# bhargav0410/gpu-accel-ofdm-ls-mrc

Hardware: AMD Instinct MI355X
Metric: OFDM symbols/s (LS+MRC) at 1024 subcarriers x 64 ant; achieved HBM GB/s vs peak (higher is better)
Workload: dtype f32; 1 GPU; OFDM uplink LS+MRC, time-domain IQ in HBM, 1250 frames x 101 symbols (1 pilot + 100 data) x 64 antennas x 1024 subcarriers per GPU; domain=time, R=64, C=1024, S=101, prefix=0, frames_per_gpu=1250, data_symbols_per_gpu=125000, global_data_symbols=125000, flow=one-launch, parallelism=frame-sharded x1, no collective

## Files before the change

### gpu-accel-ofdm-ls-mrc_amd/csrc/common.hpp

```cpp
#pragma once
#include <hip/hip_runtime.h>
#include <stdint.h>

#include "twiddles.inc"

namespace ofdm {

__constant__ __attribute__((aligned(16))) float g_twf[2 * OFDM_TW_N] = {OFDM_TW_TABLE};
#define g_tw (reinterpret_cast<const float2 *>(g_twf))
struct TwTable { float v[2 * OFDM_TW_N]; };
constexpr TwTable kTw = {{OFDM_TW_TABLE}};

template <int N, int K>
__device__ __forceinline__ constexpr float2 tw_const() {
    static_assert(OFDM_TW_N % N == 0, "N must divide 4096");
    constexpr int idx = ((K % N + N) % N) * (OFDM_TW_N / N);
    return float2{kTw.v[2 * idx], kTw.v[2 * idx + 1]};
}

__device__ __forceinline__ int lane_here() {
    int l;
    asm volatile("v_mbcnt_lo_u32_b32 %0, -1, 0\n\tv_mbcnt_hi_u32_b32 %0, -1, %0" : "=v"(l));
    return l;
}

__device__ __forceinline__ float2 cadd(float2 a, float2 b) { return {a.x + b.x, a.y + b.y}; }
__device__ __forceinline__ float2 csub(float2 a, float2 b) { return {a.x - b.x, a.y - b.y}; }
__device__ __forceinline__ float2 cmul(float2 a, float2 b) {
    return {a.x * b.x - a.y * b.y, a.x * b.y + a.y * b.x};
}
__device__ __forceinline__ float2 cconj(float2 a) { return {a.x, -a.y}; }
template <bool INV>
__device__ __forceinline__ float2 cmul_mi(float2 a) {
    return INV ? float2{-a.y, a.x} : float2{a.y, -a.x};
}
template <bool INV>
__device__ __forceinline__ float2 tw_apply(float2 a, float2 w) {
    return cmul(a, INV ? cconj(w) : w);
}

template <int N>
__device__ __forceinline__ constexpr int bitrev(int i) {
    int r = 0;
    for (int b = 1, rb = N >> 1; b < N; b <<= 1, rb >>= 1)
        if (i & b) r |= rb;
    return r;
}

template <int N, bool INV>
__device__ __forceinline__ void fft_reg(float2 (&a)[N]) {
#pragma unroll
    for (int i = 0; i < N; ++i) {
        const int j = bitrev<N>(i);
        if (i < j) { float2 t = a[i]; a[i] = a[j]; a[j] = t; }
    }
#pragma unroll
    for (int len = 2; len <= N; len <<= 1) {
        const int half = len >> 1;
#pragma unroll
        for (int i = 0; i < N; i += len) {
#pragma unroll
            for (int k = 0; k < half; ++k) {
                float2 u = a[i + k], v = a[i + k + half];
                if (k == 0) {
                } else if (4 * k == len) {
                    v = cmul_mi<INV>(v);
                } else {
                    const int idx = k * (OFDM_TW_N / len);
                    float2 w{kTw.v[2 * idx], kTw.v[2 * idx + 1]};
                    v = tw_apply<INV>(v, w);
                }
                a[i + k] = cadd(u, v);
                a[i + k + half] = csub(u, v);
            }
        }
    }
}

template <int LOG2C, bool INV>
__device__ float2 *stockham_lds(float2 *a, float2 *b) {
    constexpr int C = 1 << LOG2C;
    constexpr int TWS = OFDM_TW_N / C;
    int Ns = 1;
#pragma unroll 1
    for (; Ns * 4 <= C; Ns *= 4) {
        for (int j = threadIdx.x; j < C / 4; j += blockDim.x) {
            const int k = j & (Ns - 1);
            float2 v0 = a[j], v1 = a[j + C / 4], v2 = a[j + C / 2], v3 = a[j + 3 * C / 4];
            const int t = k * (C / (4 * Ns));
            if (t) {
                v1 = tw_apply<INV>(v1, g_tw[t * TWS]);
                v2 = tw_apply<INV>(v2, g_tw[2 * t * TWS]);
                v3 = tw_apply<INV>(v3, g_tw[3 * t * TWS]);
            }
            const float2 s02 = cadd(v0, v2), d02 = csub(v0, v2);
            const float2 s13 = cadd(v1, v3), d13 = cmul_mi<INV>(csub(v1, v3));
            const int d = (j - k) * 4 + k;
            b[d] = cadd(s02, s13);
            b[d + Ns] = cadd(d02, d13);
            b[d + 2 * Ns] = csub(s02, s13);
            b[d + 3 * Ns] = csub(d02, d13);
        }
        __syncthreads();
        float2 *t = a; a = b; b = t;
    }
    if (Ns < C) {
        for (int j = threadIdx.x; j < C / 2; j += blockDim.x) {
            const int k = j & (Ns - 1);
            float2 v0 = a[j], v1 = a[j + C / 2];
            const int t = k * (C / (2 * Ns));
            if (t) v1 = tw_apply<INV>(v1, g_tw[t * TWS]);
            const int d = (j - k) * 2 + k;
            b[d] = cadd(v0, v1);
            b[d + Ns] = csub(v0, v1);
        }
        __syncthreads();
        float2 *t = a; a = b; b = t;
    }
    return a;
}

__device__ __forceinline__ int out_pos(int j, int K) {
    const int h = (K - 1) / 2;
    return j >= h ? j - h : j + (K + 1) / 2;
}
__device__ __forceinline__ int out_pos_any(int j, int K) {
    const int h = (K - 1) / 2, n2 = (K + 1) / 2;
    return j < h ? j + n2 : (j < h + n2 ? j - h : j);
}
__device__ __forceinline__ int out_src(int k, int K) {
    const int h = (K - 1) / 2, n2 = (K + 1) / 2;
    return k < n2 ? k + h : (k < n2 + h ? k - n2 : k);
}

__device__ __forceinline__ float2 ls_conj(float2 y, float2 x) {
    const float den = x.x * x.x + x.y * x.y;
    const float rd = __builtin_amdgcn_rcpf(den);
    const float re = (y.x * x.x + y.y * x.y) * rd;
    const float im = (y.y * x.x - y.x * x.y) * rd;
    return {re, -1.0f * im};
}

__device__ __forceinline__ uint64_t splitmix64(uint64_t z) {
    z += 0x9E3779B97F4A7C15ull;
    z = (z ^ (z >> 30)) * 0xBF58476D1CE4E5B9ull;
    z = (z ^ (z >> 27)) * 0x94D049BB133111EBull;
    return z ^ (z >> 31);
}
__device__ __forceinline__ uint64_t hash4(uint64_t seed, uint64_t a, uint64_t b, uint64_t c) {
    return splitmix64(splitmix64(splitmix64(seed ^ a) ^ b) ^ c);
}
__device__ __forceinline__ float u01(uint32_t x) {
    return ((float)(x >> 8) + 1.0f) * (1.0f / 16777216.0f);
}
__device__ __forceinline__ float2 gauss2(uint64_t h) {
    const float u1 = u01((uint32_t)h), u2 = u01((uint32_t)(h >> 32));
    const float rad = sqrtf(-2.0f * logf(u1));
    float s, c;
    sincosf(6.283185307179586f * u2, &s, &c);
    return {rad * c, rad * s};
}

}
```

### gpu-accel-ofdm-ls-mrc_amd/csrc/frame_td.hip

```cpp
#include "launch.hpp"
#include "wave_fft1024.hpp"
#include "diag.hpp"

OFDM_DIAG_TU(td1024)


namespace ofdm {
namespace td1024 {

constexpr int LS_WAVES = 4;

template <int NW>
__global__ void __launch_bounds__(64 * NW) k_ls_td1024(const float2 *__restrict__ iq, int S, int R,
                                                       int prefix, const float2 *__restrict__ X,
                                                       float2 *__restrict__ Hc, float *__restrict__ P,
                                                       int partial) {
    extern __shared__ __attribute__((aligned(16))) float2 lds[];
    float2 *tw = lds;
    const int w = threadIdx.x >> 6;
    const int t = threadIdx.x & 63;
    float2 *T = lds + TWBUF + w * TBUF;
    fill_twiddles(tw);
    __syncthreads();

    const long long f = blockIdx.x;
    const int Cp = C + prefix;
    const float2 *pilot = iq + f * (long long)S * R * Cp + prefix;
    float4 *Hf = reinterpret_cast<float4 *>(Hc + f * (long long)R * C);
    const int b0 = lane_bin0(t);
    float2 xp[16];
#pragma unroll
    for (int k = 0; k < 16; ++k) {
        const int b = b0 + 16 * k;
        xp[k] = b > 0 ? X[b - 1] : float2{1.f, 0.f};
    }
    float p[16];
#pragma unroll
    for (int k = 0; k < 16; ++k) p[k] = 0.f;
    for (int r = w; r < R; r += NW) {
        float2 a[16], x[16];
        row_load(pilot + (long long)r * Cp, t, a);
        row_fft(a, t, T, tw, x);
#pragma unroll
        for (int k = 0; k < 16; ++k) {
            float2 h = ls_conj(x[k], xp[k]);
            if (b0 + 16 * k == 0) h = float2{0.f, 0.f};
            x[k] = h;
            p[k] = p[k] + (h.x * h.x) + (h.y * h.y);
        }
        hc_store(Hf + (long long)r * (C / 2), t, x);
    }
    __syncthreads();
    float *pp = reinterpret_cast<float *>(lds + TWBUF);
    static_assert(NW * C * sizeof(float) <= NW * TBUF * sizeof(float2), "partials fit the transpose images");
#pragma unroll
    for (int k = 0; k < 16; ++k) pp[w * C + b0 + 16 * k] = p[k];
    __syncthreads();
    float *Pf = P + f * C;
    const int nw = R < NW ? R : NW;
    for (int b = threadIdx.x; b < C; b += blockDim.x) {
        float sum = pp[b];
        for (int i = 1; i < nw; ++i) sum = sum + pp[i * C + b];
        Pf[b] = b == 0 ? (partial ? 0.f : 1.f) : sum;
    }
}



template <bool PREF>
__device__ __forceinline__ void hlds_row_pf(const float2 *next, const float4 *hrow, int t, float2 (&a)[16],
                                            float2 *T, const float2 *tw1, const float2 *tw2,
                                            const float4 *lo, const float4 *hi, float4 *mine,
                                            float2 (&acc)[16]) {
    using namespace hlds;
    float2 x[16];
    row_fft_a(a, t, T, tw1);
    const float4 hreg = hrow[threadIdx.x];
    __builtin_amdgcn_sched_barrier(0);
    if (PREF) row_load<true>(next, t, a);
    row_fft_b(t, T, tw2, x);
    lds_barrier();
    *mine = hreg;
    lds_barrier();
#pragma unroll
    for (int i = 0; i < 8; ++i) {
        const float4 v = i < 4 ? lo[i * 64] : hi[(i - 4) * TS];
        acc[2 * i].x = acc[2 * i].x + (x[2 * i].x * v.x - x[2 * i].y * v.y);
        acc[2 * i].y = acc[2 * i].y + (x[2 * i].x * v.y + x[2 * i].y * v.x);
        acc[2 * i + 1].x = acc[2 * i + 1].x + (x[2 * i + 1].x * v.z - x[2 * i + 1].y * v.w);
        acc[2 * i + 1].y = acc[2 * i + 1].y + (x[2 * i + 1].x * v.w + x[2 * i + 1].y * v.z);
    }
}

template <bool R0>
__device__ __forceinline__ void row0(const float2 *sym, int t, const float2 *T, float2 (&a)[16]) {
    if constexpr (R0) {
        asm volatile("s_waitcnt vmcnt(0)" ::: "memory");
#pragma unroll
        for (int m = 0; m < 16; ++m) a[m] = T[t + 64 * m];
    } else {
        row_load<true>(sym, t, a);
    }
}
__device__ __forceinline__ void row0_dma(const float2 *sym, int t, float2 *T) {
    const char *src = reinterpret_cast<const char *>(sym) + t * 16;
    const unsigned dst = lds_addr(T);
#pragma unroll
    for (int j = 0; j < 8; ++j) dma16(src + j * 1024, dst + j * 1024);
}

template <bool SHARED, bool R0 = false>
__device__ __forceinline__ void hlds_rows(const float2 *sym, int Cp, int R, const float4 *Hf, int t,
                                          float2 *T, const float2 *tw1, const float2 *tw2,
                                          float2 *T0, float4 *hfree, float2 (&acc)[16]) {
    using namespace hlds;
#pragma unroll
    for (int k = 0; k < 16; ++k) acc[k] = float2{0.f, 0.f};
    if constexpr (SHARED) {
        float2 a[16];
        row0<R0>(sym, t, T, a);
        const float4 *lo = hfree + t;
        const float4 *hi = hslot(T0, hfree, 256 + t);
        float4 *mine = hslot(T0, hfree, threadIdx.x);
        for (int r = 0; r + 1 < R; ++r)
            hlds_row_pf<true>(sym + (long long)(r + 1) * Cp, Hf + (long long)r * (C / 2), lane_here(), a, T, tw1,
                                   tw2, lo, hi, mine, acc);
        hlds_row_pf<false>(sym, Hf + (long long)(R - 1) * (C / 2), lane_here(), a, T, tw1, tw2, lo, hi, mine,
                           acc);
    } else {
        for (int r = 0; r < R; ++r) {
            float2 a[16], x[16], h[16];
            if (r == 0)
                row0<R0>(sym, t, T, a);
            else
                row_load<true>(sym + (long long)r * Cp, t, a);
            row_fft_a(a, t, T, tw1);
            row_fft_b(t, T, tw2, x);
            __builtin_amdgcn_sched_barrier(0);
            hc_load(Hf + (long long)r * (C / 2), t, h);
#pragma unroll
            for (int k = 0; k < 16; ++k) {
                acc[k].x = acc[k].x + (x[k].x * h[k].x - x[k].y * h[k].y);
                acc[k].y = acc[k].y + (x[k].x * h[k].y + x[k].y * h[k].x);
            }
        }
    }
}

__device__ __forceinline__ void hlds_epilogue(const float2 (&acc)[16], const float *P, long long f, long long q,
                                              int t, float2 *T, float2 *__restrict__ out, int mode) {
    const int b0 = lane_bin0(t);
    float2 *o = out + q * K;
    const float *Pf = P + f * C + b0;
    float pv[16];
    if ((mode & 1) == 0) {
#pragma unroll
        for (int k = 0; k < 16; ++k) pv[k] = Pf[16 * k];
    }
#pragma unroll
    for (int k = 0; k < 16; ++k) {
        const int b = b0 + 16 * k;
        float2 v = acc[k];
        int j = b - 1;
        if ((mode & 1) == 0) {
            const float rp = __builtin_amdgcn_rcpf(pv[k]);
            v = float2{acc[k].x * rp, acc[k].y * rp};
            j = out_pos(b > 0 ? b - 1 : 0, K);
        }
        if (b > 0) T[(j >> 6) * hlds::TP + (j & 63)] = v;
    }
    wave_lds_sync();
#pragma unroll
    for (int m = 0; m < 16; ++m) {
        const int j = t + 64 * m;
        if (j < K) {
            const float2 v = T[m * hlds::TP + t];
            __builtin_nontemporal_store(__builtin_bit_cast(unsigned long long, v),
                                        reinterpret_cast<unsigned long long *>(o + j));
        }
    }
}

template <bool R0>
__global__ void __attribute__((amdgpu_flat_work_group_size(512, 512), amdgpu_waves_per_eu(4, 4)))
k_mrc_td1024_hlds(const float2 *__restrict__ iq, int S, int R, int prefix, const float2 *__restrict__ Hc,
                  const float *__restrict__ P, float2 *__restrict__ out, long long nq, long long nblocks,
                  long long per_xcd, int mode) {
    using namespace hlds;
    constexpr int HW = WAVES;
    extern __shared__ __attribute__((aligned(16))) float2 lds[];
    float2 *tw1 = lds, *tw2 = lds + TW1S;
    const int w = __builtin_amdgcn_readfirstlane(threadIdx.x >> 6), t = threadIdx.x & 63;
    float2 *T = lds + TW1S + TW2S + w * TS;
    float2 *T0 = lds + TW1S + TW2S;
    float4 *hfree = reinterpret_cast<float4 *>(T0 + HW * TS);
    const long long pb = blockIdx.x;
    const long long lb = (pb & 7) * per_xcd + (pb >> 3);
    if (lb >= nblocks) return;

    const int nsym = S - 1;
    const long long qw = lb * HW + w;
    const bool store = qw < nq;
    const long long q = store ? qw : nq - 1;
    const long long f = q / nsym;
    const long long f0 = (lb * HW) / nsym;
    const long long fl = ((lb * HW + HW - 1 < nq ? lb * HW + HW - 1 : nq - 1)) / nsym;
    const int s = 1 + (int)(q % nsym);
    const int Cp = C + prefix;
    const float2 *sym = iq + (f * S + s) * (long long)R * Cp + prefix;
    if constexpr (R0) row0_dma(sym, t, T);
    fill(tw1, tw2);
    __syncthreads();

    float2 acc[16];
    if (f0 == fl)
        hlds_rows<true, R0>(sym, Cp, R, reinterpret_cast<const float4 *>(Hc + f0 * (long long)R * C), t, T,
                                 tw1, tw2, T0, hfree, acc);
    else
        hlds_rows<false, R0>(sym, Cp, R, reinterpret_cast<const float4 *>(Hc + f * (long long)R * C), t, T,
                                tw1, tw2, T0, hfree, acc);
    if (!store) return;
    hlds_epilogue(acc, P, f, q, t, T, out, mode);
}


__device__ __forceinline__ void hlds_ls_frame(const float2 *__restrict__ iq, int S, int R, int prefix,
                                              const float2 *__restrict__ X, float2 *Hc, float *P, long long f,
                                              int w, int t, float2 *T, float2 *T0, const float2 *tw1,
                                              const float2 *tw2, unsigned long long *mx = nullptr) {
    using namespace hlds;
    (void)mx;
    const int Cp = C + prefix;
    const float2 *pilot = iq + f * (long long)S * R * Cp + prefix;
    float4 *Hf = reinterpret_cast<float4 *>(Hc + f * (long long)R * C);
    const int b0 = lane_bin0(t);
    float2 xp[16];
#pragma unroll
    for (int k = 0; k < 16; ++k) {
        const int b = b0 + 16 * k;
        xp[k] = b > 0 ? X[b - 1] : float2{1.f, 0.f};
    }
    float p[16];
#pragma unroll
    for (int k = 0; k < 16; ++k) p[k] = 0.f;
    for (int r = w; r < R; r += WAVES) {
        float2 a[16], x[16];
        const int tl = lane_here();
        row_load<true>(pilot + (long long)r * Cp, tl, a);
        row_fft_a(a, tl, T, tw1);
        row_fft_b(tl, T, tw2, x);
#pragma unroll
        for (int k = 0; k < 16; ++k) {
            float2 h = ls_conj(x[k], xp[k]);
            if (b0 + 16 * k == 0) h = float2{0.f, 0.f};
            x[k] = h;
            p[k] = p[k] + (h.x * h.x) + (h.y * h.y);
        }
#pragma unroll
        for (int i = 0; i < 8; ++i) store16_wt(Hf, R * C * 8, (r * (C / 2) + i * 64 + tl) * 16, x[2 * i], x[2 * i + 1]);
        if (r == w) {
            OFDM_DIAG_MARKP(mx, 1)
        }
    }
    OFDM_DIAG_MARKP(mx, 2)
    __syncthreads();
    float *pp = reinterpret_cast<float *>(T0);
#pragma unroll
    for (int k = 0; k < 16; ++k) pp[w * C + b0 + 16 * k] = p[k];
    __syncthreads();
    float *Pf = P + f * C;
    const int nw = R < WAVES ? R : WAVES;
    for (int b = threadIdx.x; b < C; b += blockDim.x) {
        float sum = pp[b];
        for (int i = 1; i < nw; ++i) sum = sum + pp[i * C + b];
        const float v = b == 0 ? 1.f : sum;
        store4_wt(Pf + b, v);
    }
    OFDM_DIAG_MARKP(mx, 3)
    __syncthreads();
}

__device__ __forceinline__ void split_unit(const float2 *__restrict__ iq, int S, int R, int prefix, const float2 *Hc,
                                           const float *P, float2 *__restrict__ out, long long nq, long long q0, int w,
                                           int t, float2 *T, float2 *T0, const float2 *tw1, const float2 *tw2) {
    const int nsym = S - 1, Cp = C + prefix, hh = w >> 2, R0 = (R + 1) >> 1;
    const long long qw = q0 + (w & 3);
    const bool store = qw < nq;
    const long long q = store ? qw : nq - 1;
    const long long f = q / nsym;
    const int s = 1 + (int)(q % nsym);
    const float2 *sym = iq + (f * S + s) * (long long)R * Cp + prefix;
    const float4 *Hf = reinterpret_cast<const float4 *>(Hc + f * (long long)R * C);
    float2 acc[16];
#pragma unroll
    for (int k = 0; k < 16; ++k) acc[k] = float2{0.f, 0.f};
    const int r1 = hh ? R : R0;
    for (int r = hh ? R0 : 0; r < r1; ++r) {
        float2 a[16], x[16], h[16];
        row_load<true>(sym + (long long)r * Cp, t, a);
        hlds::row_fft_a(a, t, T, tw1);
        hlds::row_fft_b(t, T, tw2, x);
        __builtin_amdgcn_sched_barrier(0);
        hc_load(Hf + (long long)r * (C / 2), t, h);
#pragma unroll
        for (int k = 0; k < 16; ++k) {
            acc[k].x = acc[k].x + (x[k].x * h[k].x - x[k].y * h[k].y);
            acc[k].y = acc[k].y + (x[k].x * h[k].y + x[k].y * h[k].x);
        }
    }
    if (hh) {
#pragma unroll
        for (int k = 0; k < 16; ++k) T[k * hlds::TP + t] = acc[k];
    }
    __syncthreads();
    if (hh) return;
    const float2 *Tp = T0 + (w + 4) * hlds::TS;
#pragma unroll
    for (int k = 0; k < 16; ++k) {
        const float2 v = Tp[k * hlds::TP + t];
        acc[k] = float2{acc[k].x + v.x, acc[k].y + v.y};
    }
    if (store) hlds_epilogue(acc, P, f, q, t, T, out, 0);
}

__global__ void __attribute__((amdgpu_flat_work_group_size(512, 512), amdgpu_waves_per_eu(4, 4)))
k_demod_td1024(const float2 *__restrict__ iq, int S, int R, int prefix, const float2 *__restrict__ X, float2 *Hc,
               float *P, float2 *__restrict__ out, long long nq, long long nblocks, Tickets tk, long long k0, long long split, unsigned long long *flags, unsigned long long epoch,
               int nls, long long nframes, long long spin_ticks) {
    using namespace hlds;
    constexpr int HW = WAVES;
    extern __shared__ __attribute__((aligned(16))) float2 lds[];
    float2 *tw1 = lds, *tw2 = lds + TW1S;
    const int w = __builtin_amdgcn_readfirstlane(threadIdx.x >> 6), t = threadIdx.x & 63;
    float2 *T = lds + TW1S + TW2S + w * TS;
    float2 *T0 = lds + TW1S + TW2S;
    float4 *hfree = reinterpret_cast<float4 *>(T0 + HW * TS);
    OFDM_DIAG_BEGIN()

    const bool estimator = (int)blockIdx.x < nls;
    auto first_frame = [&](long long lb) { return (lb * HW) / (S - 1); };
    auto last_frame = [&](long long lb) { return ((lb * HW + HW - 1 < nq ? lb * HW + HW - 1 : nq - 1)) / (S - 1); };
    const int nsym = S - 1, Cp = C + prefix;
    auto sym_of = [&](long long lb) {
        const long long qw = lb * HW + w, q = qw < nq ? qw : nq - 1;
        return iq + ((q / nsym) * S + 1 + q % nsym) * (long long)R * Cp + prefix;
    };
    long long e0 = 1, e1 = 0, lb = 0;
    int um = 0;
    if (estimator) {
        e0 = e1 = blockIdx.x;
        if (e0 >= nframes) return;
        __builtin_amdgcn_s_setprio(3);
        fill(tw1, tw2);
        __syncthreads();
        OFDM_DIAG_MARKN(0)
    } else {
        FillRegs fr;
        fill_load(fr);
        lb = wg_take_unit(tk, nblocks, k0, (long long)blockIdx.x - nls, split,
                          reinterpret_cast<long long *>(hfree + 255));
        if (lb < 0) return;
        OFDM_DIAG_MARKN(0)
        um = (int)(lb & 3);
        lb >>= 2;
        fill_store(tw1, tw2, fr);
        const long long f0 = first_frame(lb), fl = last_frame(lb);
        if (!um) row0_dma(sym_of(lb), t, T);
        bool seen_before = false;
        if (threadIdx.x == 0)
            seen_before = __hip_atomic_load((gu64 *)(flags + f0), __ATOMIC_RELAXED, __HIP_MEMORY_SCOPE_AGENT) == epoch &&
                          __hip_atomic_load((gu64 *)(flags + fl), __ATOMIC_RELAXED, __HIP_MEMORY_SCOPE_AGENT) == epoch;
        OFDM_DIAG_MARKN(1)
        if (!consume_flags(flags, f0, fl, epoch, spin_ticks, reinterpret_cast<int *>(hfree), seen_before)) {
            asm volatile("s_waitcnt vmcnt(0)" ::: "memory");
            __syncthreads();
            e0 = f0;
            e1 = fl;
        }
    }
    for (long long ff = e0; ff <= e1; ++ff)
        hlds_ls_frame(iq, S, R, prefix, X, Hc, P, ff, w, t, T, T0, tw1, tw2, OFDM_DIAG_ARG);
    if (estimator) {
        OFDM_DIAG_MARK()
        publish_flag(flags + e0, epoch);
        OFDM_DIAG_END_SLOT(td1024, epoch);
        return;
    }
    if (e0 <= e1) {
        acquire_all();
        if (!um) row0_dma(sym_of(lb), t, T);
    }
    OFDM_DIAG_MARK()

    if (um) {
        split_unit(iq, S, R, prefix, Hc, P, out, nq, lb * HW + 4 * (um - 1), w, t, T, T0, tw1, tw2);
        OFDM_DIAG_END_SLOT(td1024, epoch);
        return;
    }
    const long long qw = lb * HW + w;
    const bool store = qw < nq;
    const long long q = store ? qw : nq - 1;
    const long long f = q / nsym;
    const long long f0 = first_frame(lb), fl = last_frame(lb);
    const float2 *sym = sym_of(lb);
    float2 acc[16];
    if (f0 == fl)
        hlds_rows<true, true>(sym, Cp, R, reinterpret_cast<const float4 *>(Hc + f0 * (long long)R * C), t, T,
                              tw1, tw2, T0, hfree, acc);
    else
        hlds_rows<false, true>(sym, Cp, R, reinterpret_cast<const float4 *>(Hc + f * (long long)R * C), t, T,
                               tw1, tw2, T0, hfree, acc);
    OFDM_DIAG_MARKN(2)
    if (store) hlds_epilogue(acc, P, f, q, lane_here(), T, out, 0);
    OFDM_DIAG_END_SLOT(td1024, epoch);
}

}

hipError_t launch_ls_td1024(const float2 *iq, long long nframes, int S, int R, int prefix,
                            const float2 *X, float2 *Hc, float *P, int partial, hipStream_t s) {
    using namespace td1024;
    if (nframes <= 0) return hipSuccess;
    if (nframes > 0x7fffffffll) return hipErrorInvalidValue;
    int nw = (nframes * LS_WAVES < 2048 && R > LS_WAVES) ? 16 : LS_WAVES;
    auto k16 = k_ls_td1024<16>;
    auto k4 = k_ls_td1024<LS_WAVES>;
    auto k8 = k16;
    if (nw == 16 || nw == 8) {
        auto kern = nw == 16 ? k16 : k8;
        const size_t lds = (TWBUF + nw * TBUF) * sizeof(float2);
        if (hipError_t e = opt_in_lds(reinterpret_cast<const void *>(kern), (int)lds); e != hipSuccess) return e;
        hipLaunchKernelGGL(kern, dim3((unsigned)nframes), dim3(64 * nw), lds, s, iq, S, R, prefix, X, Hc, P,
                           partial);
        return hipGetLastError();
    }
    const size_t lds = (TWBUF + LS_WAVES * TBUF) * sizeof(float2);
    hipLaunchKernelGGL(k4, dim3((unsigned)nframes), dim3(64 * LS_WAVES), lds, s, iq, S, R, prefix, X, Hc, P,
                       partial);
    return hipGetLastError();
}

hipError_t launch_mrc_td1024(const float2 *iq, long long nframes, int S, int R, int prefix,
                             const float2 *Hc, const float *P, float2 *out, int mode,
                             hipStream_t s) {
    using namespace td1024;
    const long long nq = nframes * (S - 1);
    if (nq <= 0) return hipSuccess;
    const long long nb = (nq + hlds::WAVES - 1) / hlds::WAVES;
    const long long pxcd = (nb + 7) / 8;
    if (pxcd * 8 > 0x7fffffffll) return hipErrorInvalidValue;
    auto kern = k_mrc_td1024_hlds<true>;
    hipLaunchKernelGGL(kern, dim3((unsigned)(pxcd * 8)), dim3(64 * hlds::WAVES), hlds::LDS_BYTES, s, iq, S, R,
                       prefix, Hc, P, out, nq, nb, pxcd, mode);
    return hipGetLastError();
}

hipError_t launch_demod_td1024(const float2 *iq, long long nframes, int S, int R, int prefix, const float2 *X,
                               float2 *Hc, float *P, float2 *out, Tickets tk,
                               unsigned long long *flags, unsigned long long epoch, long long spin_ticks,
                               hipStream_t s) {
    using namespace td1024;
    const long long nq = nframes * (S - 1);
    if (nq <= 0) return hipSuccess;
    const long long nb = (nq + hlds::WAVES - 1) / hlds::WAVES;
    const long long nls = (nframes + 7) / 8 * 8;
    const long long k1 = ticket_k0(2), k0 = 2 * k1, split = R >= 2 ? k1 : 0;
    const long long g = ticket_grid(nb, 8 * split);
    if (g + nls > 0x7fffffffll) return hipErrorInvalidValue;
    hipLaunchKernelGGL(k_demod_td1024, dim3((unsigned)(nls + g)), dim3(64 * hlds::WAVES), hlds::LDS_BYTES, s, iq,
                       S, R, prefix, X, Hc, P, out, nq, nb, tk, k0, split, flags, epoch, (int)nls, nframes,
                       spin_ticks < 0 ? SPIN_TICKS : spin_ticks);
    return hipGetLastError();
}

}
```

### gpu-accel-ofdm-ls-mrc_amd/csrc/wave_fft1024.hpp

```cpp
#pragma once
#include "common.hpp"
#include "launch.hpp"
#include "pk.hpp"

namespace ofdm {
namespace td1024 {

constexpr int C = 1024;
constexpr int K = C - 1;
constexpr int TP = 68;
constexpr int TBUF = 16 * TP;
constexpr int TW1P = 17;
constexpr int TW1BUF = 64 * TW1P;
constexpr int TW2P = 17;
constexpr int TW2BUF = 4 * TW2P;
constexpr int TWBUF = TW1BUF + TW2BUF;

__device__ __forceinline__ void wave_lds_sync() {
    __builtin_amdgcn_fence(__ATOMIC_RELEASE, "wavefront");
    __builtin_amdgcn_wave_barrier();
    __builtin_amdgcn_fence(__ATOMIC_ACQUIRE, "wavefront");
}

__device__ __forceinline__ void lds_barrier() {
    asm volatile("s_waitcnt lgkmcnt(0)\n\ts_barrier" ::: "memory");
}

typedef __attribute__((address_space(3))) void lvoid_t;
__device__ __forceinline__ unsigned lds_addr(const void *p) { return (unsigned)(size_t)(lvoid_t *)p; }

__device__ __forceinline__ void dma16(const void *g, unsigned lds) {
    unsigned keep;
    asm volatile("s_mov_b32 %0, m0\n\ts_mov_b32 m0, %2\n\ts_nop 0\n\tglobal_load_lds_dwordx4 %1, off\n\t"
                 "s_mov_b32 m0, %0"
                 : "=&s"(keep)
                 : "v"(g), "s"(lds)
                 : "memory");
}

__device__ __forceinline__ float quad_g(int a) { return (a == 0 || a == 3) ? 1.f : -1.f; }

__device__ __forceinline__ void fill_twiddles(float2 *tw) {
    for (int i = threadIdx.x; i < TW1BUF; i += blockDim.x) {
        const int t = i / TW1P, k2 = i % TW1P;
        tw[i] = k2 < 16 ? g_tw[((t * k2) & (C - 1)) * (OFDM_TW_N / C)] : float2{0.f, 0.f};
    }
    for (int i = threadIdx.x; i < TW2BUF; i += blockDim.x) {
        const int a = i / TW2P, k = i % TW2P;
        const float2 w = g_tw[((16 * a * k) & (C - 1)) * (OFDM_TW_N / C)];
        const float g = quad_g(a);
        tw[TW1BUF + i] = k < 16 ? float2{g * w.x, g * w.y} : float2{0.f, 0.f};
    }
}

template <int CTRL>
__device__ __forceinline__ float dpp(float v) {
    return __builtin_bit_cast(float, __builtin_amdgcn_mov_dpp(__builtin_bit_cast(int, v), CTRL,
                                                              0xF, 0xF, true));
}
constexpr int DPP_XOR1 = 0xB1;
constexpr int DPP_XOR2 = 0x4E;

template <bool NT = false>
__device__ __forceinline__ void row_load(const float2 *__restrict__ src, int t, float2 (&a)[16]) {
    if (NT) {
        const unsigned long long *p = reinterpret_cast<const unsigned long long *>(src) + t;
#pragma unroll
        for (int m = 0; m < 16; ++m)
            a[m] = __builtin_bit_cast(float2, __builtin_nontemporal_load(p + 64 * m));
    } else {
#pragma unroll
        for (int m = 0; m < 16; ++m) a[m] = src[t + 64 * m];
    }
}

#define OFDM_DPP_Q(CTRL) "quad_perm:" CTRL " row_mask:0xf bank_mask:0xf"
template <int CTRL>
__device__ __forceinline__ void quad_fmac_dpp(float (&v)[16], float S) {
#define OFDM_F(i) "v_fmac_f32_dpp %" #i ", %" #i ", %16 " OFDM_DPP_Q(QP) "\n\t"
    if constexpr (CTRL == 0x4E) {
#define QP "[2,3,0,1]"
        asm("s_nop 1\n\t" OFDM_F(0) OFDM_F(1) OFDM_F(2) OFDM_F(3) OFDM_F(4) OFDM_F(5) OFDM_F(6)
                OFDM_F(7) OFDM_F(8) OFDM_F(9) OFDM_F(10) OFDM_F(11) OFDM_F(12) OFDM_F(13) OFDM_F(14)
                    OFDM_F(15)
            : "+v"(v[0]), "+v"(v[1]), "+v"(v[2]), "+v"(v[3]), "+v"(v[4]), "+v"(v[5]), "+v"(v[6]),
              "+v"(v[7]), "+v"(v[8]), "+v"(v[9]), "+v"(v[10]), "+v"(v[11]), "+v"(v[12]),
              "+v"(v[13]), "+v"(v[14]), "+v"(v[15])
            : "v"(S));
#undef QP
    } else {
        static_assert(CTRL == 0xB1, "quad xor 1 or xor 2");
#define QP "[1,0,3,2]"
        asm("s_nop 1\n\t" OFDM_F(0) OFDM_F(1) OFDM_F(2) OFDM_F(3) OFDM_F(4) OFDM_F(5) OFDM_F(6)
                OFDM_F(7) OFDM_F(8) OFDM_F(9) OFDM_F(10) OFDM_F(11) OFDM_F(12) OFDM_F(13) OFDM_F(14)
                    OFDM_F(15)
            : "+v"(v[0]), "+v"(v[1]), "+v"(v[2]), "+v"(v[3]), "+v"(v[4]), "+v"(v[5]), "+v"(v[6]),
              "+v"(v[7]), "+v"(v[8]), "+v"(v[9]), "+v"(v[10]), "+v"(v[11]), "+v"(v[12]),
              "+v"(v[13]), "+v"(v[14]), "+v"(v[15])
            : "v"(S));
#undef QP
    }
#undef OFDM_F
}
#undef OFDM_DPP_Q

__device__ __forceinline__ void quad_dft(float2 (&x)[16], int qa) {
    const float S1 = (qa & 2) ? 1.f : -1.f;
    const float S2 = (qa & 1) ? 1.f : -1.f;
    const unsigned long long rot = __builtin_amdgcn_ballot_w64(qa == 3);
    float xr[16], xi[16];
#pragma unroll
    for (int k = 0; k < 16; ++k) { xr[k] = x[k].x; xi[k] = x[k].y; }
    quad_fmac_dpp<DPP_XOR2>(xr, S1);
    quad_fmac_dpp<DPP_XOR2>(xi, S1);
#pragma unroll
    for (int k = 0; k < 16; ++k) {
        float nx;
        asm("v_cndmask_b32_e64 %0, %2, %3, %4\n\tv_cndmask_b32_e64 %1, %3, -%2, %4"
            : "=&v"(nx), "=v"(xi[k])
            : "v"(xr[k]), "v"(xi[k]), "s"(rot));
        xr[k] = nx;
    }
    quad_fmac_dpp<DPP_XOR1>(xr, S2);
    quad_fmac_dpp<DPP_XOR1>(xi, S2);
#pragma unroll
    for (int k = 0; k < 16; ++k) x[k] = float2{xr[k], xi[k]};
}

__device__ __forceinline__ void row_fft(float2 (&a)[16], int t, float2 *T, const float2 *tw,
                                        float2 (&x)[16]) {
    fft_reg<16, false>(a);
#pragma unroll
    for (int k2 = 1; k2 < 16; ++k2) a[k2] = cmul(a[k2], tw[t * TW1P + k2]);
#pragma unroll
    for (int k2 = 0; k2 < 16; ++k2) T[k2 * TP + t] = a[k2];
    wave_lds_sync();
    const int q = t >> 2, qa = t & 3;
#pragma unroll
    for (int l = 0; l < 16; ++l) x[l] = T[q * TP + qa + 4 * l];
    wave_lds_sync();
    fft_reg<16, false>(x);
    const float2 *tw2 = tw + TW1BUF + qa * TW2P;
    const float g = quad_g(qa);
    x[0] = float2{g * x[0].x, g * x[0].y};
#pragma unroll
    for (int k = 1; k < 16; ++k) x[k] = cmul(x[k], tw2[k]);
    quad_dft(x, qa);
}

__device__ __forceinline__ int lane_bin0(int t) {
    const int qa = t & 3;
    return (t >> 2) + 256 * ((qa >> 1) + 2 * (qa & 1));
}

__device__ __forceinline__ void hc_store(float4 *__restrict__ dst, int t, const float2 (&h)[16]) {
#pragma unroll
    for (int i = 0; i < 8; ++i)
        dst[i * 64 + t] = float4{h[2 * i].x, h[2 * i].y, h[2 * i + 1].x, h[2 * i + 1].y};
}
__device__ __forceinline__ void hc_load(const float4 *__restrict__ src, int t, float2 (&h)[16]) {
#pragma unroll
    for (int i = 0; i < 8; ++i) {
        const float4 v = src[i * 64 + t];
        h[2 * i] = float2{v.x, v.y};
        h[2 * i + 1] = float2{v.z, v.w};
    }
}

typedef __attribute__((address_space(1))) unsigned long long gu64;
typedef __attribute__((address_space(1))) unsigned gu32;
constexpr long long SPIN_TICKS = 200000;

__device__ __forceinline__ void store16_wt(const void *base, int bytes, int off, float2 a, float2 b) {
    typedef int v4i __attribute__((ext_vector_type(4)));
    const __amdgpu_buffer_rsrc_t rs =
        __builtin_amdgcn_make_buffer_rsrc(const_cast<void *>(base), (short)0, bytes, 0x00020000);
    const v4i v = {__builtin_bit_cast(int, a.x), __builtin_bit_cast(int, a.y), __builtin_bit_cast(int, b.x),
                   __builtin_bit_cast(int, b.y)};
    __builtin_amdgcn_raw_buffer_store_b128(v, rs, off, 0, 16);
}
__device__ __forceinline__ void store8_wt(float2 *p, float2 v) {
    __hip_atomic_store((gu64 *)(p), __builtin_bit_cast(unsigned long long, v), __ATOMIC_RELAXED,
                       __HIP_MEMORY_SCOPE_AGENT);
}
__device__ __forceinline__ void store4_wt(float *p, float v) {
    __hip_atomic_store((gu32 *)(p), __builtin_bit_cast(unsigned, v), __ATOMIC_RELAXED, __HIP_MEMORY_SCOPE_AGENT);
}

__device__ __forceinline__ void publish_flag(unsigned long long *flag, unsigned long long epoch) {
    asm volatile("s_waitcnt vmcnt(0)" ::: "memory");
    __syncthreads();
    if (threadIdx.x == 0) {
        asm volatile("s_waitcnt vmcnt(0)" ::: "memory");
        __hip_atomic_store((gu64 *)(flag), epoch, __ATOMIC_RELAXED, __HIP_MEMORY_SCOPE_AGENT);
    }
}

__device__ __forceinline__ bool wait_flag(unsigned long long *flag, unsigned long long epoch, long long ticks) {
    const long long t0 = wall_clock64();
    while (__hip_atomic_load((gu64 *)(flag), __ATOMIC_RELAXED, __HIP_MEMORY_SCOPE_AGENT) != epoch) {
        if (wall_clock64() - t0 >= ticks) return false;
        __builtin_amdgcn_s_sleep(2);
    }
    return true;
}

__device__ __forceinline__ bool consume_flags(unsigned long long *flags, long long f0, long long fl,
                                              unsigned long long epoch, long long ticks, int *seen,
                                              bool seen_before = false) {
    if (threadIdx.x == 0) {
        bool ok = true;
        if (!seen_before)
            for (long long f = f0; f <= fl && ok; ++f) ok = wait_flag(flags + f, epoch, ticks);
        *seen = ok ? 1 : 0;
        if (ok) __builtin_amdgcn_fence(__ATOMIC_ACQUIRE, "agent");
        asm volatile("s_waitcnt vmcnt(0)" ::: "memory");
    }
    __syncthreads();
    const bool ok = *seen != 0;
    __syncthreads();
    return ok;
}
__device__ __forceinline__ void acquire_all() {
    asm volatile("s_waitcnt vmcnt(0)" ::: "memory");
    __syncthreads();
    if (threadIdx.x == 0) {
        __builtin_amdgcn_fence(__ATOMIC_ACQUIRE, "agent");
        asm volatile("s_waitcnt vmcnt(0)" ::: "memory");
    }
    __syncthreads();
}

constexpr int TICKET_STRIDE = 16;
constexpr int HWREG_XCC_ID = (31 << 11) | 20;
__device__ __forceinline__ long long ticket_range_count(long long nb, long long per, unsigned y) {
    const long long lo = (long long)y * per;
    return nb - lo < per ? (nb - lo > 0 ? nb - lo : 0) : per;
}
__device__ __forceinline__ void ticket_fault(const Tickets &tk, unsigned why) {
    if (tk.status) __hip_atomic_store((gu32 *)tk.status, why, __ATOMIC_RELAXED, __HIP_MEMORY_SCOPE_SYSTEM);
}
__device__ __forceinline__ long long take_ticket(const Tickets &tk, unsigned y, long long units) {
    gu64 *p = (gu64 *)(tk.set + y * TICKET_STRIDE);
    const unsigned long long mine = (unsigned long long)tk.tag << 32;
    unsigned long long v = __hip_atomic_load(p, __ATOMIC_RELAXED, __HIP_MEMORY_SCOPE_AGENT);
    for (int tries = 0; (v >> 32) != tk.tag; ++tries) {
        if (tries == 64) {
            ticket_fault(tk, TK_CONTENDED);
            return -2;
        }
        if (__hip_atomic_compare_exchange_strong(p, &v, mine | 1ull, __ATOMIC_RELAXED, __ATOMIC_RELAXED,
                                                 __HIP_MEMORY_SCOPE_AGENT))
            return 0;
    }
    if ((long long)(unsigned)v >= units) return -1;
    const unsigned long long r = __hip_atomic_fetch_add(p, 1ull, __ATOMIC_RELAXED, __HIP_MEMORY_SCOPE_AGENT);
    if ((r >> 32) != tk.tag) {
        ticket_fault(tk, TK_FOREIGN);
        return -2;
    }
    const long long t = (long long)(unsigned)r;
    if (t < units) return t;
    if (t > units + (long long)gridDim.x) ticket_fault(tk, TK_RANGE);
    return -1;
}
__device__ __forceinline__ long long take_unit(const Tickets &tk, long long nb, long long k0, long long pb,
                                               long long split) {
    const long long per = (nb + 7) / 8;
    if (pb < 8 * k0) {
        const unsigned y = (unsigned)(pb & 7);
        const long long k = pb >> 3, cnt = ticket_range_count(nb, per, y);
        if (k < (cnt < k0 ? cnt : k0)) return ((long long)y * per + k) << 2;
    }
    const unsigned x = (unsigned)__builtin_amdgcn_s_getreg(HWREG_XCC_ID) & 7u;
    for (int j = 0; j < 8; ++j) {
        const unsigned y = (x + (unsigned)j) & 7u;
        const long long cnt = ticket_range_count(nb, per, y), s0 = cnt < k0 ? cnt : k0;
        const long long avail = cnt - s0;
        if (avail <= 0) continue;
        const long long ns = split < avail ? split : avail, whole = avail - ns;
        const long long t = take_ticket(tk, y, whole + 2 * ns);
        if (t < 0) continue;
        const long long b0 = (long long)y * per + s0;
        if (t < whole) return (b0 + t) << 2;
        const long long u = t - whole;
        return ((b0 + whole + (u >> 1)) << 2) | (1 + (u & 1));
    }
    return -1;
}
__device__ __forceinline__ long long wg_take_unit(const Tickets &tk, long long nb, long long k0, long long pb,
                                                  long long split, long long *slot) {
    if (threadIdx.x == 0) {
        if (pb == 0) {
#pragma unroll
            for (int y = 0; y < 8; ++y)
                __hip_atomic_store((gu64 *)(tk.set + y * TICKET_STRIDE), (unsigned long long)tk.tag << 32,
                                   __ATOMIC_RELAXED, __HIP_MEMORY_SCOPE_AGENT);
        }
        *slot = take_unit(tk, nb, k0, pb, split);
    }
    __syncthreads();
    const long long v = *slot;
    const int lo = __builtin_amdgcn_readfirstlane((int)(v & 0xffffffffll));
    const int hi = __builtin_amdgcn_readfirstlane((int)(v >> 32));
    return (long long)(((unsigned long long)(unsigned)hi << 32) | (unsigned)lo);
}
__device__ __forceinline__ long long wg_take_block(const Tickets &tk, long long nb, long long k0, long long pb,
                                                   long long *slot) {
    const long long u = wg_take_unit(tk, nb, k0, pb, 0, slot);
    return u < 0 ? u : u >> 2;
}
inline long long ticket_grid(long long nb, long long split_units = 0) { return nb + split_units + nb / 4 + 64; }
inline long long ticket_k0(int per_cu) {
    static const int cus = [] {
        int dev = 0, n = 256;
        if (hipGetDevice(&dev) != hipSuccess || hipDeviceGetAttribute(&n, hipDeviceAttributeMultiprocessorCount, dev) != hipSuccess)
            n = 256;
        return n;
    }();
    return (long long)per_cu * cus / 8;
}

namespace hlds {
constexpr int TW1S = 15 * 64;
constexpr int TW2S = 16 * 4;
constexpr int TP = 68;
constexpr int TS = 16 * TP;
constexpr int WAVES = 8;
constexpr size_t LDS_BYTES = (TW1S + TW2S + WAVES * TS) * sizeof(float2) + 256 * sizeof(float4);
static_assert(LDS_BYTES == 81920, "two workgroups per CU");

__device__ __forceinline__ float4 *hslot(float2 *T0, float4 *hfree, int j) {
    if (j < 256) return hfree + j;
    const int jj = j - 256;
    return reinterpret_cast<float4 *>(T0 + (jj >> 5) * TS + ((jj >> 1) & 15) * TP + 64 + 2 * (jj & 1));
}

__device__ __forceinline__ void fill(float2 *tw1, float2 *tw2) {
    for (int i = threadIdx.x; i < TW1S; i += blockDim.x) {
        const int k2 = 1 + i / 64, t = i % 64;
        tw1[i] = g_tw[((t * k2) & (C - 1)) * (OFDM_TW_N / C)];
    }
    for (int i = threadIdx.x; i < TW2S; i += blockDim.x) {
        const int k = i / 4, a = i % 4;
        const float2 w = g_tw[((16 * a * k) & (C - 1)) * (OFDM_TW_N / C)];
        const float g = quad_g(a);
        tw2[i] = float2{g * w.x, g * w.y};
    }
}
struct FillRegs {
    float2 v[3];
};
__device__ __forceinline__ void fill_load(FillRegs &f) {
    const int i0 = threadIdx.x, i1 = threadIdx.x + 512;
    auto w1 = [](int i) { return g_tw[(((i % 64) * (1 + i / 64)) & (C - 1)) * (OFDM_TW_N / C)]; };
    f.v[0] = w1(i0);
    f.v[1] = i1 < TW1S ? w1(i1) : float2{0.f, 0.f};
    f.v[2] = i0 < TW2S ? g_tw[((16 * (i0 % 4) * (i0 / 4)) & (C - 1)) * (OFDM_TW_N / C)] : float2{0.f, 0.f};
}
__device__ __forceinline__ void fill_store(float2 *tw1, float2 *tw2, const FillRegs &f) {
    const int i0 = threadIdx.x, i1 = threadIdx.x + 512;
    tw1[i0] = f.v[0];
    if (i1 < TW1S) tw1[i1] = f.v[1];
    if (i0 < TW2S) {
        const float g = quad_g(i0 % 4);
        tw2[i0] = float2{g * f.v[2].x, g * f.v[2].y};
    }
}
static_assert(TW1S <= 1024 && TW2S <= 512, "fill_load covers the tables with 512 threads");
__device__ __forceinline__ int swz(int row, int col) { return row * TP + col; }

template <int N>
__device__ __forceinline__ void tw_powers(pk::v2f (&v)[N], pk::v2f w, pk::v2f sw) {
    const pk::v2f w2 = pk::cmul(w, w);
    pk::v2f po = sw, pe = pk::cmul(sw, w);
    v[1] = pk::cmul(v[1], po);
    v[2] = pk::cmul(v[2], pe);
#pragma unroll
    for (int k = 3; k < N; k += 2) {
        po = pk::cmul(po, w2);
        v[k] = pk::cmul(v[k], po);
        if (k + 1 < N) {
            pe = pk::cmul(pe, w2);
            v[k + 1] = pk::cmul(v[k + 1], pe);
        }
    }
}

template <int PK = 0, bool TWR = false>
__device__ __forceinline__ void row_fft_a(float2 (&a)[16], int t, float2 *T, const float2 *tw1) {
    if constexpr (TWR) {
        pk::v2f v[16];
#pragma unroll
        for (int m = 0; m < 16; ++m) v[m] = pk::V(a[m]);
        if constexpr ((PK & 1) != 0) {
            pk::fft_reg<16>(v);
        } else {
#pragma unroll
            for (int m = 0; m < 16; ++m) a[m] = pk::F(v[m]);
            fft_reg<16, false>(a);
#pragma unroll
            for (int m = 0; m < 16; ++m) v[m] = pk::V(a[m]);
        }
        const pk::v2f w = pk::V(tw1[t]);
        tw_powers(v, w, w);
#pragma unroll
        for (int k2 = 0; k2 < 16; ++k2) T[swz(k2, t)] = pk::F(v[k2]);
        return;
    }
    if constexpr (PK & 1) {
        pk::v2f v[16];
#pragma unroll
        for (int m = 0; m < 16; ++m) v[m] = pk::V(a[m]);
        pk::fft_reg<16>(v);
#pragma unroll
        for (int k2 = 1; k2 < 16; ++k2) v[k2] = pk::cmul(v[k2], pk::V(tw1[(k2 - 1) * 64 + t]));
#pragma unroll
        for (int k2 = 0; k2 < 16; ++k2) T[swz(k2, t)] = pk::F(v[k2]);
        return;
    }
    fft_reg<16, false>(a);
#pragma unroll
    for (int k2 = 1; k2 < 16; ++k2) a[k2] = cmul(a[k2], tw1[(k2 - 1) * 64 + t]);
#pragma unroll
    for (int k2 = 0; k2 < 16; ++k2) T[swz(k2, t)] = a[k2];
}
template <int PK = 0, bool TWR = false>
__device__ __forceinline__ void row_fft_b(int t, float2 *T, const float2 *tw2, float2 (&x)[16]) {
    wave_lds_sync();
    const int q = t >> 2, qa = t & 3;
#pragma unroll
    for (int l = 0; l < 16; ++l) x[l] = T[swz(q, qa + 4 * l)];
    wave_lds_sync();
    const float g = quad_g(qa);
    if constexpr (TWR) {
        pk::v2f v[16];
        if constexpr ((PK & 2) != 0) {
#pragma unroll
            for (int m = 0; m < 16; ++m) v[m] = pk::V(x[m]);
            pk::fft_reg<16>(v);
        } else {
            fft_reg<16, false>(x);
#pragma unroll
            for (int m = 0; m < 16; ++m) v[m] = pk::V(x[m]);
        }
        v[0] = pk::scale(v[0], g);
        const pk::v2f gw = pk::V(tw2[4 + qa]);
        tw_powers(v, pk::scale(gw, g), gw);
#pragma unroll
        for (int m = 0; m < 16; ++m) x[m] = pk::F(v[m]);
    } else if constexpr (PK & 2) {
        pk::v2f v[16];
#pragma unroll
        for (int m = 0; m < 16; ++m) v[m] = pk::V(x[m]);
        pk::fft_reg<16>(v);
        v[0] = pk::scale(v[0], g);
#pragma unroll
        for (int k = 1; k < 16; ++k) v[k] = pk::cmul(v[k], pk::V(tw2[k * 4 + qa]));
#pragma unroll
        for (int m = 0; m < 16; ++m) x[m] = pk::F(v[m]);
    } else {
        fft_reg<16, false>(x);
        x[0] = float2{g * x[0].x, g * x[0].y};
#pragma unroll
        for (int k = 1; k < 16; ++k) x[k] = cmul(x[k], tw2[k * 4 + qa]);
    }
    quad_dft(x, qa);
}
constexpr int TP16 = 72;
constexpr int TS16 = 16 * TP16;
__device__ __forceinline__ int perm16(int c) { return 8 * (c >> 3) + 2 * (c & 3) + ((c >> 2) & 1); }
__device__ __forceinline__ void fa_write16(const pk::v2f (&v)[16], int pt, float2 *T) {
#pragma unroll
    for (int k2 = 0; k2 < 16; ++k2) T[k2 * TP16 + pt] = pk::F(v[k2]);
}
__device__ __forceinline__ void fb_read16(int t, const float2 *T, pk::v2f (&v)[16]) {
    const float4 *s = reinterpret_cast<const float4 *>(T + (t >> 2) * TP16 + 2 * (t & 3));
#pragma unroll
    for (int j = 0; j < 8; ++j) {
        const float4 x = s[4 * j];
        v[2 * j] = pk::V(float2{x.x, x.y});
        v[2 * j + 1] = pk::V(float2{x.z, x.w});
    }
}

struct TwAnchors {
    pk::v2f w, a1, a4, a8, a12;
};
__device__ __forceinline__ void tw_anchored(pk::v2f (&v)[16], const TwAnchors &c) {
    const pk::v2f w2 = pk::cmul(c.w, c.w), w3 = pk::cmul(w2, c.w);
    v[1] = pk::cmul(v[1], c.a1);
    v[2] = pk::cmul(v[2], pk::cmul(c.a1, c.w));
    v[3] = pk::cmul(v[3], pk::cmul(c.a1, w2));
#pragma unroll
    for (int j = 1; j < 4; ++j) {
        const pk::v2f a = j == 1 ? c.a4 : j == 2 ? c.a8 : c.a12;
        v[4 * j] = pk::cmul(v[4 * j], a);
        v[4 * j + 1] = pk::cmul(v[4 * j + 1], pk::cmul(a, c.w));
        v[4 * j + 2] = pk::cmul(v[4 * j + 2], pk::cmul(a, w2));
        v[4 * j + 3] = pk::cmul(v[4 * j + 3], pk::cmul(a, w3));
    }
}
__device__ __forceinline__ TwAnchors anchors_a(const float2 *tw1, int t) {
    const pk::v2f w = pk::V(tw1[t]);
    return TwAnchors{w, w, pk::V(tw1[3 * 64 + t]), pk::V(tw1[7 * 64 + t]), pk::V(tw1[11 * 64 + t])};
}
__device__ __forceinline__ TwAnchors anchors_b(const float2 *tw2, int t) {
    const int qa = t & 3;
    const pk::v2f gw = pk::V(tw2[4 + qa]);
    return TwAnchors{pk::scale(gw, quad_g(qa)), gw, pk::V(tw2[16 + qa]), pk::V(tw2[32 + qa]), pk::V(tw2[48 + qa])};
}

__device__ __forceinline__ void fa_compute(pk::v2f (&v)[16], pk::v2f w1) {
    pk::fft_reg<16>(v);
    tw_powers(v, w1, w1);
}
__device__ __forceinline__ void fa_compute(pk::v2f (&v)[16], const TwAnchors &c) {
    pk::fft_reg<16>(v);
    tw_anchored(v, c);
}
__device__ __forceinline__ void fa_write(const pk::v2f (&v)[16], int t, float2 *T) {
#pragma unroll
    for (int k2 = 0; k2 < 16; ++k2) T[swz(k2, t)] = pk::F(v[k2]);
}
__device__ __forceinline__ void fb_read(int t, const float2 *T, pk::v2f (&v)[16]) {
    const int q = t >> 2, qa = t & 3;
#pragma unroll
    for (int l = 0; l < 16; ++l) v[l] = pk::V(T[swz(q, qa + 4 * l)]);
}
__device__ __forceinline__ void fb_compute(pk::v2f (&v)[16], pk::v2f gw, int t, float2 (&x)[16]) {
    const int qa = t & 3;
    const float g = quad_g(qa);
    pk::fft_reg<16>(v);
    v[0] = pk::scale(v[0], g);
    tw_powers(v, pk::scale(gw, g), gw);
#pragma unroll
    for (int m = 0; m < 16; ++m) x[m] = pk::F(v[m]);
    quad_dft(x, qa);
}
__device__ __forceinline__ void fb_compute(pk::v2f (&v)[16], const TwAnchors &c, int t, float2 (&x)[16]) {
    const int qa = t & 3;
    pk::fft_reg<16>(v);
    v[0] = pk::scale(v[0], quad_g(qa));
    tw_anchored(v, c);
#pragma unroll
    for (int m = 0; m < 16; ++m) x[m] = pk::F(v[m]);
    quad_dft(x, qa);
}

}

}
}
```

Measured before the change: 10.17 million symbols/s.

## Use FMA-factored radix-16 butterflies, buffer loads for H, and wave-uniform indices

Adds an FFT-16 variant that factors each twiddle multiply into a ratio-plus-FMA form (Linzer-Feig style) and routes the row FFT paths through it. MAC accumulations are rewritten as explicit FMA chains. The shared-H path now loads channel rows through a raw buffer resource with wave-uniform offsets, and frame index plus flag publishing are made wave-uniform via readfirstlane. The goal is fewer VALU ops and less scalar/vector address math per row, at the cost of slightly different rounding in the FFT.

```diff
diff --git a/gpu-accel-ofdm-ls-mrc_amd/csrc/common.hpp b/gpu-accel-ofdm-ls-mrc_amd/csrc/common.hpp
--- a/gpu-accel-ofdm-ls-mrc_amd/csrc/common.hpp
+++ b/gpu-accel-ofdm-ls-mrc_amd/csrc/common.hpp
@@ -72,6 +72,51 @@
                 }
                 a[i + k] = cadd(u, v);
                 a[i + k + half] = csub(u, v);
+            }
+        }
+    }
+}
+
+__device__ __forceinline__ void fft16_fma(float2 (&a)[16]) {
+    constexpr int N = 16;
+#pragma unroll
+    for (int i = 0; i < N; ++i) {
+        const int j = bitrev<N>(i);
+        if (i < j) { float2 t = a[i]; a[i] = a[j]; a[j] = t; }
+    }
+#pragma unroll
+    for (int len = 2; len <= N; len <<= 1) {
+        const int half = len >> 1;
+#pragma unroll
+        for (int i = 0; i < N; i += len) {
+#pragma unroll
+            for (int k = 0; k < half; ++k) {
+                const float2 u = a[i + k], v = a[i + k + half];
+                if (k == 0 || 4 * k == len) {
+                    const float2 p = k == 0 ? v : cmul_mi<false>(v);
+                    a[i + k] = cadd(u, p);
+                    a[i + k + half] = csub(u, p);
+                    continue;
+                }
+                const int idx = k * (OFDM_TW_N / len);
+                const float c = kTw.v[2 * idx], s = kTw.v[2 * idx + 1];
+                const float ac = c < 0.f ? -c : c, as = s < 0.f ? -s : s;
+                float2 p;
+                float m;
+                if (ac == as) {
+                    p = c == s ? float2{v.x - v.y, v.y + v.x} : float2{v.x + v.y, v.y - v.x};
+                    m = c;
+                } else if (ac > as) {
+                    const float t = s / c;
+                    p = float2{__builtin_fmaf(-t, v.y, v.x), __builtin_fmaf(t, v.x, v.y)};
+                    m = c;
+                } else {
+                    const float t = c / s;
+                    p = float2{__builtin_fmaf(t, v.x, -v.y), __builtin_fmaf(t, v.y, v.x)};
+                    m = s;
+                }
+                a[i + k] = float2{__builtin_fmaf(m, p.x, u.x), __builtin_fmaf(m, p.y, u.y)};
+                a[i + k + half] = float2{__builtin_fmaf(-m, p.x, u.x), __builtin_fmaf(-m, p.y, u.y)};
             }
         }
     }
diff --git a/gpu-accel-ofdm-ls-mrc_amd/csrc/frame_td.hip b/gpu-accel-ofdm-ls-mrc_amd/csrc/frame_td.hip
--- a/gpu-accel-ofdm-ls-mrc_amd/csrc/frame_td.hip
+++ b/gpu-accel-ofdm-ls-mrc_amd/csrc/frame_td.hip
@@ -66,29 +66,40 @@
 }
 
 
-
+__device__ __forceinline__ void fft_a(float2 (&a)[16], int t, float2 *T, const float2 *tw1) {
+    hlds::row_fft_a<0, false, true>(a, t, T, tw1);
+}
+__device__ __forceinline__ void fft_b(int t, float2 *T, const float2 *tw2, float2 (&x)[16]) {
+    hlds::row_fft_b<0, false, true>(t, T, tw2, x);
+}
+__device__ __forceinline__ void mac(float2 &acc, float2 x, float vx, float vy) {
+    acc.x = __builtin_fmaf(-x.y, vy, __builtin_fmaf(x.x, vx, acc.x));
+    acc.y = __builtin_fmaf(x.y, vx, __builtin_fmaf(x.x, vy, acc.y));
+}
+
+
+typedef int v4i_t __attribute__((ext_vector_type(4)));
 template <bool PREF>
-__device__ __forceinline__ void hlds_row_pf(const float2 *next, const float4 *hrow, int t, float2 (&a)[16],
+__device__ __forceinline__ void hlds_row_pf(const float2 *next, __amdgpu_buffer_rsrc_t hc, int hoff, int t,
+                                            float2 (&a)[16],
                                             float2 *T, const float2 *tw1, const float2 *tw2,
                                             const float4 *lo, const float4 *hi, float4 *mine,
                                             float2 (&acc)[16]) {
     using namespace hlds;
     float2 x[16];
-    row_fft_a(a, t, T, tw1);
-    const float4 hreg = hrow[threadIdx.x];
+    fft_a(a, t, T, tw1);
+    const float4 hreg = __builtin_bit_cast(float4, (v4i_t)__builtin_amdgcn_raw_buffer_load_b128(hc, t * 16, hoff, 0));
     __builtin_amdgcn_sched_barrier(0);
     if (PREF) row_load<true>(next, t, a);
-    row_fft_b(t, T, tw2, x);
+    fft_b(t, T, tw2, x);
     lds_barrier();
     *mine = hreg;
     lds_barrier();
 #pragma unroll
     for (int i = 0; i < 8; ++i) {
         const float4 v = i < 4 ? lo[i * 64] : hi[(i - 4) * TS];
-        acc[2 * i].x = acc[2 * i].x + (x[2 * i].x * v.x - x[2 * i].y * v.y);
-        acc[2 * i].y = acc[2 * i].y + (x[2 * i].x * v.y + x[2 * i].y * v.x);
-        acc[2 * i + 1].x = acc[2 * i + 1].x + (x[2 * i + 1].x * v.z - x[2 * i + 1].y * v.w);
-        acc[2 * i + 1].y = acc[2 * i + 1].y + (x[2 * i + 1].x * v.w + x[2 * i + 1].y * v.z);
+        mac(acc[2 * i], x[2 * i], v.x, v.y);
+        mac(acc[2 * i + 1], x[2 * i + 1], v.z, v.w);
     }
 }
 
@@ -118,15 +129,18 @@
     for (int k = 0; k < 16; ++k) acc[k] = float2{0.f, 0.f};
     if constexpr (SHARED) {
         float2 a[16];
-        row0<R0>(sym, t, T, a);
-        const float4 *lo = hfree + t;
-        const float4 *hi = hslot(T0, hfree, 256 + t);
+        const int tl = lane_here();
+        row0<R0>(sym, tl, T, a);
+        const float4 *lo = hfree + tl;
+        const float4 *hi = hslot(T0, hfree, 256 + tl);
         float4 *mine = hslot(T0, hfree, threadIdx.x);
+        const __amdgpu_buffer_rsrc_t hc =
+            __builtin_amdgcn_make_buffer_rsrc(const_cast<float4 *>(Hf), (short)0, R * (C * 8), 0x00020000);
+        const int hw = __builtin_amdgcn_readfirstlane(threadIdx.x >> 6) * 1024;
         for (int r = 0; r + 1 < R; ++r)
-            hlds_row_pf<true>(sym + (long long)(r + 1) * Cp, Hf + (long long)r * (C / 2), lane_here(), a, T, tw1,
-                                   tw2, lo, hi, mine, acc);
-        hlds_row_pf<false>(sym, Hf + (long long)(R - 1) * (C / 2), lane_here(), a, T, tw1, tw2, lo, hi, mine,
-                           acc);
+            hlds_row_pf<true>(sym + (long long)(r + 1) * Cp, hc, r * (C * 8) + hw, lane_here(), a, T, tw1, tw2, lo,
+                              hi, mine, acc);
+        hlds_row_pf<false>(sym, hc, (R - 1) * (C * 8) + hw, lane_here(), a, T, tw1, tw2, lo, hi, mine, acc);
     } else {
         for (int r = 0; r < R; ++r) {
             float2 a[16], x[16], h[16];
@@ -134,15 +148,12 @@
                 row0<R0>(sym, t, T, a);
             else
                 row_load<true>(sym + (long long)r * Cp, t, a);
-            row_fft_a(a, t, T, tw1);
-            row_fft_b(t, T, tw2, x);
+            fft_a(a, t, T, tw1);
+            fft_b(t, T, tw2, x);
             __builtin_amdgcn_sched_barrier(0);
             hc_load(Hf + (long long)r * (C / 2), t, h);
 #pragma unroll
-            for (int k = 0; k < 16; ++k) {
-                acc[k].x = acc[k].x + (x[k].x * h[k].x - x[k].y * h[k].y);
-                acc[k].y = acc[k].y + (x[k].x * h[k].y + x[k].y * h[k].x);
-            }
+            for (int k = 0; k < 16; ++k) mac(acc[k], x[k], h[k].x, h[k].y);
         }
     }
 }
@@ -202,7 +213,7 @@
     const long long qw = lb * HW + w;
     const bool store = qw < nq;
     const long long q = store ? qw : nq - 1;
-    const long long f = q / nsym;
+    const long long f = uniform64(q / nsym);
     const long long f0 = (lb * HW) / nsym;
     const long long fl = ((lb * HW + HW - 1 < nq ? lb * HW + HW - 1 : nq - 1)) / nsym;
     const int s = 1 + (int)(q % nsym);
@@ -220,7 +231,7 @@
         hlds_rows<false, R0>(sym, Cp, R, reinterpret_cast<const float4 *>(Hc + f * (long long)R * C), t, T,
                                 tw1, tw2, T0, hfree, acc);
     if (!store) return;
-    hlds_epilogue(acc, P, f, q, t, T, out, mode);
+    hlds_epilogue(acc, P, f, q, lane_here(), T, out, mode);
 }
 
 
@@ -247,8 +258,8 @@
         float2 a[16], x[16];
         const int tl = lane_here();
         row_load<true>(pilot + (long long)r * Cp, tl, a);
-        row_fft_a(a, tl, T, tw1);
-        row_fft_b(tl, T, tw2, x);
+        fft_a(a, tl, T, tw1);
+        fft_b(tl, T, tw2, x);
 #pragma unroll
         for (int k = 0; k < 16; ++k) {
             float2 h = ls_conj(x[k], xp[k]);
@@ -298,15 +309,12 @@
     for (int r = hh ? R0 : 0; r < r1; ++r) {
         float2 a[16], x[16], h[16];
         row_load<true>(sym + (long long)r * Cp, t, a);
-        hlds::row_fft_a(a, t, T, tw1);
-        hlds::row_fft_b(t, T, tw2, x);
+        fft_a(a, t, T, tw1);
+        fft_b(t, T, tw2, x);
         __builtin_amdgcn_sched_barrier(0);
         hc_load(Hf + (long long)r * (C / 2), t, h);
 #pragma unroll
-        for (int k = 0; k < 16; ++k) {
-            acc[k].x = acc[k].x + (x[k].x * h[k].x - x[k].y * h[k].y);
-            acc[k].y = acc[k].y + (x[k].x * h[k].y + x[k].y * h[k].x);
-        }
+        for (int k = 0; k < 16; ++k) mac(acc[k], x[k], h[k].x, h[k].y);
     }
     if (hh) {
 #pragma unroll
@@ -382,7 +390,7 @@
         hlds_ls_frame(iq, S, R, prefix, X, Hc, P, ff, w, t, T, T0, tw1, tw2, OFDM_DIAG_ARG);
     if (estimator) {
         OFDM_DIAG_MARK()
-        publish_flag(flags + e0, epoch);
+        publish_flag(flags + e0, epoch, w == 0 && lane_here() == 0);
         OFDM_DIAG_END_SLOT(td1024, epoch);
         return;
     }
diff --git a/gpu-accel-ofdm-ls-mrc_amd/csrc/wave_fft1024.hpp b/gpu-accel-ofdm-ls-mrc_amd/csrc/wave_fft1024.hpp
--- a/gpu-accel-ofdm-ls-mrc_amd/csrc/wave_fft1024.hpp
+++ b/gpu-accel-ofdm-ls-mrc_amd/csrc/wave_fft1024.hpp
@@ -129,7 +129,7 @@
 
 __device__ __forceinline__ void row_fft(float2 (&a)[16], int t, float2 *T, const float2 *tw,
                                         float2 (&x)[16]) {
-    fft_reg<16, false>(a);
+    fft16_fma(a);
 #pragma unroll
     for (int k2 = 1; k2 < 16; ++k2) a[k2] = cmul(a[k2], tw[t * TW1P + k2]);
 #pragma unroll
@@ -139,7 +139,7 @@
 #pragma unroll
     for (int l = 0; l < 16; ++l) x[l] = T[q * TP + qa + 4 * l];
     wave_lds_sync();
-    fft_reg<16, false>(x);
+    fft16_fma(x);
     const float2 *tw2 = tw + TW1BUF + qa * TW2P;
     const float g = quad_g(qa);
     x[0] = float2{g * x[0].x, g * x[0].y};
@@ -187,10 +187,10 @@
     __hip_atomic_store((gu32 *)(p), __builtin_bit_cast(unsigned, v), __ATOMIC_RELAXED, __HIP_MEMORY_SCOPE_AGENT);
 }
 
-__device__ __forceinline__ void publish_flag(unsigned long long *flag, unsigned long long epoch) {
+__device__ __forceinline__ void publish_flag(unsigned long long *flag, unsigned long long epoch, bool one) {
     asm volatile("s_waitcnt vmcnt(0)" ::: "memory");
     __syncthreads();
-    if (threadIdx.x == 0) {
+    if (one) {
         asm volatile("s_waitcnt vmcnt(0)" ::: "memory");
         __hip_atomic_store((gu64 *)(flag), epoch, __ATOMIC_RELAXED, __HIP_MEMORY_SCOPE_AGENT);
     }
@@ -263,6 +263,11 @@
     if (t < units) return t;
     if (t > units + (long long)gridDim.x) ticket_fault(tk, TK_RANGE);
     return -1;
+}
+__device__ __forceinline__ long long uniform64(long long v) {
+    const int lo = __builtin_amdgcn_readfirstlane((int)(v & 0xffffffffll));
+    const int hi = __builtin_amdgcn_readfirstlane((int)(v >> 32));
+    return (long long)(((unsigned long long)(unsigned)hi << 32) | (unsigned)lo);
 }
 __device__ __forceinline__ long long take_unit(const Tickets &tk, long long nb, long long k0, long long pb,
                                                long long split) {
@@ -301,9 +306,7 @@
     }
     __syncthreads();
     const long long v = *slot;
-    const int lo = __builtin_amdgcn_readfirstlane((int)(v & 0xffffffffll));
-    const int hi = __builtin_amdgcn_readfirstlane((int)(v >> 32));
-    return (long long)(((unsigned long long)(unsigned)hi << 32) | (unsigned)lo);
+    return uniform64(v);
 }
 __device__ __forceinline__ long long wg_take_block(const Tickets &tk, long long nb, long long k0, long long pb,
                                                    long long *slot) {
@@ -387,7 +390,7 @@
     }
 }
 
-template <int PK = 0, bool TWR = false>
+template <int PK = 0, bool TWR = false, bool FMA = false>
 __device__ __forceinline__ void row_fft_a(float2 (&a)[16], int t, float2 *T, const float2 *tw1) {
     if constexpr (TWR) {
         pk::v2f v[16];
@@ -419,13 +422,17 @@
         for (int k2 = 0; k2 < 16; ++k2) T[swz(k2, t)] = pk::F(v[k2]);
         return;
     }
-    fft_reg<16, false>(a);
+    static_assert(!FMA || (PK == 0 && !TWR), "fft16_fma is the plain-f32 table-twiddle path's");
+    if constexpr (FMA)
+        fft16_fma(a);
+    else
+        fft_reg<16, false>(a);
 #pragma unroll
     for (int k2 = 1; k2 < 16; ++k2) a[k2] = cmul(a[k2], tw1[(k2 - 1) * 64 + t]);
 #pragma unroll
     for (int k2 = 0; k2 < 16; ++k2) T[swz(k2, t)] = a[k2];
 }
-template <int PK = 0, bool TWR = false>
+template <int PK = 0, bool TWR = false, bool FMA = false>
 __device__ __forceinline__ void row_fft_b(int t, float2 *T, const float2 *tw2, float2 (&x)[16]) {
     wave_lds_sync();
     const int q = t >> 2, qa = t & 3;
@@ -460,7 +467,11 @@
 #pragma unroll
         for (int m = 0; m < 16; ++m) x[m] = pk::F(v[m]);
     } else {
-        fft_reg<16, false>(x);
+        static_assert(!FMA || (PK == 0 && !TWR), "fft16_fma is the plain-f32 table-twiddle path's");
+        if constexpr (FMA)
+            fft16_fma(x);
+        else
+            fft_reg<16, false>(x);
         x[0] = float2{g * x[0].x, g * x[0].y};
 #pragma unroll
         for (int k = 1; k < 16; ++k) x[k] = cmul(x[k], tw2[k * 4 + qa]);
```

Result: faster. 10.43 million symbols/s (median of 6 runs) (+2.5%).
